# guy3540/Acoustic_Locating_VQ-VAE

Measured on AMD Instinct MI355X. Metric: spectrograms/sec (train step), speech VQ-VAE default config, higher is better.
Workload: dtype x3mx_hb

## Files before the change

acoustic_locating_vq-vae_amd/csrc/vq.hip:

```cpp
#include "alvq_common.h"

namespace alvq {

constexpr int VQ_RB_MAX = 128;
constexpr int VQ_CT = 128;
constexpr int VQ_DK = 32;
constexpr int VQ_ES = 34;
constexpr int VQ_PARTIALS = 1024;

__host__ __device__ constexpr int vq_pad32(int x, int r) { return x + ((r - x % 32) + 32) % 32; }

__global__ __launch_bounds__(256) void row_sqnorm_kernel(const float* x, float* out, long rows, int D) {
  const int lane = threadIdx.x & 63;
  for (long r = (long)blockIdx.x * 4 + (threadIdx.x >> 6); r < rows; r += (long)gridDim.x * 4) {
    float s = 0.f;
    for (int d = lane; d < D; d += 64) {
      const float v = x[r * D + d];
      s += v * v;
    }
    s = wave_sum(s);
    if (lane == 0) out[r] = s;
  }
}

struct ArgminArgs {
  const float* x;
  const float* e;
  const float* xn;
  const float* en;
  int64_t* idx;
  float* min_dist;
  long N;
  int K, D, Dp, XSTR;
};

template <int NW>
__global__ __launch_bounds__(64 * NW, 2) void vq_argmin_f32_kernel(ArgminArgs a) {
  constexpr int NT = 64 * NW, VQ_RB = 16 * NW, EPT = VQ_CT * VQ_DK / NT, ERS = NT / 32;
  extern __shared__ __attribute__((aligned(16))) float smem[];
  float* Xs = smem;
  float* Es = smem + VQ_RB * a.XSTR;

  const int tid = threadIdx.x, lane = tid & 63, wave = tid >> 6;
  const int li = lane & 15, kq = lane >> 4;
  const long r0 = (long)blockIdx.x * VQ_RB;
  const int D = a.D, K = a.K, XSTR = a.XSTR;

  for (int e = tid; e < VQ_RB * a.Dp; e += NT) {
    const int r = e / a.Dp, d = e - r * a.Dp;
    const long row = r0 + r;
    Xs[r * XSTR + d] = (row < a.N && d < D) ? a.x[row * D + d] : 0.f;
  }

  float xn[4];
#pragma unroll
  for (int r = 0; r < 4; ++r) {
    const long row = r0 + wave * 16 + kq * 4 + r;
    xn[r] = row < a.N ? a.xn[row] : 0.f;
  }
  float best[4];
  int bidx[4];
#pragma unroll
  for (int r = 0; r < 4; ++r) {
    best[r] = __builtin_inff();
    bidx[r] = 0x7fffffff;
  }

  const int ecol = tid & 31, erow0 = tid >> 5;
  float er[EPT];
  auto load_e = [&](int k0, int d0) {
#pragma unroll
    for (int i = 0; i < EPT; ++i) {
      const int k = k0 + erow0 + ERS * i, d = d0 + ecol;
      er[i] = (k < K && d < D) ? a.e[(long)k * D + d] : 0.f;
    }
  };
  auto store_e = [&]() {
#pragma unroll
    for (int i = 0; i < EPT; ++i) Es[(erow0 + ERS * i) * VQ_ES + ecol] = er[i];
  };

  const int nd = a.Dp / VQ_DK;
  const int nkt = (K + VQ_CT - 1) / VQ_CT;
  const int total = nkt * nd;
  load_e(0, 0);
  store_e();
  __syncthreads();
  f32x4 acc[8];
  for (int it = 0; it < total; ++it) {
    const int kt = it / nd, dc = it - kt * nd;
    if (dc == 0) {
#pragma unroll
      for (int ni = 0; ni < 8; ++ni) acc[ni] = f32x4{0.f, 0.f, 0.f, 0.f};
    }
    if (it + 1 < total) {
      const int kt2 = (it + 1) / nd, dc2 = (it + 1) - kt2 * nd;
      load_e(kt2 * VQ_CT, dc2 * VQ_DK);
    }
#pragma unroll
    for (int s = 0; s < VQ_DK / 4; ++s) {
      const float af = Xs[(wave * 16 + li) * XSTR + dc * VQ_DK + s * 4 + kq];
#pragma unroll
      for (int ni = 0; ni < 8; ++ni) {
        const float bf = Es[(ni * 16 + li) * VQ_ES + s * 4 + kq];
        acc[ni] = __builtin_amdgcn_mfma_f32_16x16x4f32(af, bf, acc[ni], 0, 0, 0);
      }
    }
    if (dc == nd - 1) {
#pragma unroll
      for (int ni = 0; ni < 8; ++ni) {
        const int k = kt * VQ_CT + ni * 16 + li;
        if (k < K) {
          const float bn = a.en[k];
#pragma unroll
          for (int r = 0; r < 4; ++r) {
            const float d = (xn[r] + bn) - 2.0f * acc[ni][r];
            if (d < best[r]) {
              best[r] = d;
              bidx[r] = k;
            }
          }
        }
      }
    }
    __syncthreads();
    if (it + 1 < total) {
      store_e();
      __syncthreads();
    }
  }

#pragma unroll
  for (int o = 1; o < 16; o <<= 1) {
#pragma unroll
    for (int r = 0; r < 4; ++r) {
      const float d2 = __shfl_xor(best[r], o, 64);
      const int k2 = __shfl_xor(bidx[r], o, 64);
      if (d2 < best[r] || (d2 == best[r] && k2 < bidx[r])) {
        best[r] = d2;
        bidx[r] = k2;
      }
    }
  }
  if (li == 0) {
#pragma unroll
    for (int r = 0; r < 4; ++r) {
      const long row = r0 + wave * 16 + kq * 4 + r;
      if (row < a.N) {
        a.idx[row] = (int64_t)(bidx[r] == 0x7fffffff ? 0 : bidx[r]);
        if (a.min_dist) a.min_dist[row] = best[r];
      }
    }
  }
}

constexpr int VQR_ES = 36;
template <int ND, int RW>
__global__ __launch_bounds__(256, (ND == 8 && RW == 1) ? 3 : 2) void vq_argmin_f32_reg_kernel(ArgminArgs a) {
  __shared__ __attribute__((aligned(16))) float Es[2][VQ_CT * VQR_ES];
  const int tid = threadIdx.x, lane = tid & 63, wave = tid >> 6;
  const int li = lane & 15, kq = lane >> 4;
  const long r0 = (long)blockIdx.x * (64 * RW) + wave * (16 * RW);
  const int D = a.D, K = a.K;
  const bool vec = (D & 3) == 0;

  float xa[RW][ND * 8];
#pragma unroll
  for (int f = 0; f < RW; ++f) {
    const long row = r0 + f * 16 + li;
    const float* xr = a.x + row * D;
#pragma unroll
    for (int j = 0; j < ND * 8; ++j) {
      const int d = 4 * j + kq;
      xa[f][j] = (row < a.N && d < D) ? xr[d] : 0.f;
    }
  }
  float xn[RW][4], best[RW][4];
  int bidx[RW][4];
#pragma unroll
  for (int f = 0; f < RW; ++f)
#pragma unroll
    for (int r = 0; r < 4; ++r) {
      const long row = r0 + f * 16 + kq * 4 + r;
      xn[f][r] = row < a.N ? a.xn[row] : 0.f;
      best[f][r] = __builtin_inff();
      bidx[f][r] = 0x7fffffff;
    }

  const int c8 = tid & 7, ecode = tid >> 3;
  f32x4 er[4];
  auto load_e = [&](int kt, int dc) {
#pragma unroll
    for (int i = 0; i < 4; ++i) {
      const int k = kt * VQ_CT + ecode + 32 * i, d = dc * VQ_DK + 4 * c8;
      const float* p = a.e + (long)k * D + d;
      if (k < K && vec && d + 3 < D) er[i] = *(const f32x4*)p;
      else {
#pragma unroll
        for (int q = 0; q < 4; ++q) er[i][q] = (k < K && d + q < D) ? p[q] : 0.f;
      }
    }
  };
  auto store_e = [&](int buf) {
#pragma unroll
    for (int i = 0; i < 4; ++i)
#pragma unroll
      for (int q = 0; q < 4; ++q) Es[buf][(ecode + 32 * i) * VQR_ES + q * 8 + c8] = er[i][q];
  };

  const int nkt = (K + VQ_CT - 1) / VQ_CT;
  load_e(0, 0);
  store_e(0);
  __syncthreads();
  for (int kt = 0; kt < nkt; ++kt) {
    f32x4 acc[RW][8];
#pragma unroll
    for (int f = 0; f < RW; ++f)
#pragma unroll
      for (int ni = 0; ni < 8; ++ni) acc[f][ni] = f32x4{0.f, 0.f, 0.f, 0.f};
#pragma unroll
    for (int dc = 0; dc < ND; ++dc) {
      const bool more = !(kt == nkt - 1 && dc == ND - 1);
      if (more) load_e(dc == ND - 1 ? kt + 1 : kt, dc == ND - 1 ? 0 : dc + 1);
      const float* eb = &Es[dc & 1][li * VQR_ES + kq * 8];
#pragma unroll
      for (int half = 0; half < 2; ++half) {
        f32x4 b0[4], b1[4];
#pragma unroll
        for (int n4 = 0; n4 < 4; ++n4) {
          const float* p = eb + (half * 4 + n4) * 16 * VQR_ES;
          b0[n4] = *(const f32x4*)p;
          b1[n4] = *(const f32x4*)(p + 4);
        }
#pragma unroll
        for (int s = 0; s < 8; ++s)
#pragma unroll
          for (int n4 = 0; n4 < 4; ++n4) {
            const float bf = s < 4 ? b0[n4][s & 3] : b1[n4][s & 3];
#pragma unroll
            for (int f = 0; f < RW; ++f)
              acc[f][half * 4 + n4] = __builtin_amdgcn_mfma_f32_16x16x4f32(xa[f][dc * 8 + s], bf, acc[f][half * 4 + n4], 0, 0, 0);
          }
      }
      if (more) store_e((dc + 1) & 1);
      __syncthreads();
    }
#pragma unroll
    for (int ni = 0; ni < 8; ++ni) {
      const int k = kt * VQ_CT + ni * 16 + li;
      if (k < K) {
        const float bn = a.en[k];
#pragma unroll
        for (int f = 0; f < RW; ++f)
#pragma unroll
          for (int r = 0; r < 4; ++r) {
            const float d = (xn[f][r] + bn) - 2.0f * acc[f][ni][r];
            if (d < best[f][r]) {
              best[f][r] = d;
              bidx[f][r] = k;
            }
          }
      }
    }
  }
#pragma unroll
  for (int o = 1; o < 16; o <<= 1)
#pragma unroll
    for (int f = 0; f < RW; ++f)
#pragma unroll
      for (int r = 0; r < 4; ++r) {
        const float d2 = __shfl_xor(best[f][r], o, 64);
        const int k2 = __shfl_xor(bidx[f][r], o, 64);
        if (d2 < best[f][r] || (d2 == best[f][r] && k2 < bidx[f][r])) {
          best[f][r] = d2;
          bidx[f][r] = k2;
        }
      }
  if (li == 0) {
#pragma unroll
    for (int f = 0; f < RW; ++f)
#pragma unroll
      for (int r = 0; r < 4; ++r) {
        const long row = r0 + f * 16 + kq * 4 + r;
        if (row < a.N) {
          a.idx[row] = (int64_t)(bidx[f][r] == 0x7fffffff ? 0 : bidx[f][r]);
          if (a.min_dist) a.min_dist[row] = best[f][r];
        }
      }
  }
}

__global__ __launch_bounds__(256) void vq_gather_loss_kernel(const float* x, const float* e, const int64_t* idx,
                                                             float* q_st, float* partials, int32_t* hist, long N, int K,
                                                             int D) {
  const int lane = threadIdx.x & 63, wave = threadIdx.x >> 6;
  extern __shared__ int lhist[];
  const bool use_lds = hist && K <= 8192;
  if (use_lds) {
    for (int k = threadIdx.x; k < K; k += 256) lhist[k] = 0;
    __syncthreads();
  }
  const long per = (N + gridDim.x - 1) / gridDim.x;
  const long rb = (long)blockIdx.x * per, re = rb + per < N ? rb + per : N;
  float s = 0.f;
  for (long r = rb + wave; r < re; r += 4) {
    const long k = idx[r];
    for (int d = lane; d < D; d += 64) {
      const float xv = x[r * D + d];
      const float diff = e[k * D + d] - xv;
      q_st[r * D + d] = xv + diff;
      s += diff * diff;
    }
    if (lane == 0 && hist) atomicAdd(use_lds ? &lhist[k] : &hist[k], 1);
  }
  if (use_lds) {
    __syncthreads();
    for (int k = threadIdx.x; k < K; k += 256)
      if (lhist[k]) atomicAdd(&hist[k], lhist[k]);
  }
  __shared__ float red[4];
  s = block_sum<kPairwise4, false>(s, red);
  if (threadIdx.x == 0) partials[blockIdx.x] = s;
}

template <bool QLAT>
__global__ __launch_bounds__(256) void vq_finalize_kernel(const float* partials, int nparts, const int32_t* hist,
                                                          float* out, long N, int K, int D, float beta) {
  __shared__ float red[256];
  const int t = threadIdx.x;
  float s = 0.f;
  for (int i = t; i < nparts; i += 256) s += partials[i];
  const float sq = tree256_sum<true>(s, red);
  float h = 0.f;
  for (int k = t; k < K; k += 256) {
    const float p = (float)hist[k] / (float)N;
    h += p * logf(p + 1e-10f);
  }
  h = tree256_sum<false>(h, red);
  if (t == 0) {
    const float m = sq / (float)((double)N * (double)D);
    out[0] = QLAT ? m + beta * m : beta * m;
    out[1] = expf(-h);
  }
}

__global__ __launch_bounds__(256) void vq_backward_dx_kernel(const float* g, const float* grad_loss, const float* x,
                                                             const float* e, const int64_t* idx, float* dx, long N, int D,
                                                             float cx) {
  const int lane = threadIdx.x & 63, wave = threadIdx.x >> 6;
  const float sx = (grad_loss ? grad_loss[0] : 1.f) * cx;
  for (long r = (long)blockIdx.x * 4 + wave; r < N; r += (long)gridDim.x * 4) {
    const long k = idx[r];
    for (int d = lane; d < D; d += 64) {
      const float diff = e[k * D + d] - x[r * D + d];
      dx[r * D + d] = (g ? g[r * D + d] : 0.f) - sx * diff;
    }
  }
}

constexpr int VQL_CAP = 2048;
constexpr int VQL_CHUNK = 1024;
template <int VEC>
__global__ __launch_bounds__(256) void vq_codebook_grad_kernel(const float* grad_loss, const float* x, const float* e,
                                                               const int64_t* idx, float* partial, long N, int K, int D,
                                                               long rows_per_part, float ce) {
  typedef float vec_t __attribute__((ext_vector_type(VEC)));
  __shared__ int list[VQL_CAP];
  __shared__ int wave_tot[4];
  __shared__ vec_t comb[256];
  const int k = blockIdx.x, part = blockIdx.y, tid = threadIdx.x;
  const float se = (grad_loss ? grad_loss[0] : 1.f) * ce;
  const int TD = D / VEC;
  const int G = 256 / TD;
  const int grp = tid / TD, ld = tid - grp * TD;
  const bool summer = grp < G;
  vec_t ek, acc;
#pragma unroll
  for (int v = 0; v < VEC; ++v) {
    ek[v] = summer ? e[(long)k * D + ld * VEC + v] : 0.f;
    acc[v] = 0.f;
  }
  int nlist = 0;
  auto flush = [&]() {
    if (!summer) return;
    int i = grp;
    for (; i + G < nlist; i += 2 * G) {
      const vec_t a = *(const vec_t*)(x + (long)list[i] * D + ld * VEC);
      const vec_t b = *(const vec_t*)(x + (long)list[i + G] * D + ld * VEC);
      acc += se * (ek - a);
      acc += se * (ek - b);
    }
    if (i < nlist) acc += se * (ek - *(const vec_t*)(x + (long)list[i] * D + ld * VEC));
  };
  const long rbeg = (long)part * rows_per_part;
  const long rend = rbeg + rows_per_part < N ? rbeg + rows_per_part : N;
  for (long base = rbeg; base < rend; base += VQL_CHUNK) {
    int mine[4], cnt = 0;
#pragma unroll
    for (int j = 0; j < 4; ++j) {
      const long r = base + 4 * tid + j;
      if (r < rend && idx[r] == k) mine[cnt++] = (int)r;
    }
    int total;
    const int pos = nlist + block_scan_excl<false>(cnt, wave_tot, total);
    for (int j = 0; j < cnt; ++j) list[pos + j] = mine[j];
    nlist += total;
    __syncthreads();
    if (nlist > VQL_CAP - VQL_CHUNK) {
      flush();
      nlist = 0;
      __syncthreads();
    }
  }
  flush();
  comb[tid] = acc;
  __syncthreads();
  if (tid < TD) {
    vec_t s = comb[tid];
    for (int g = 1; g < G; ++g) s += comb[g * TD + tid];
    *(vec_t*)(partial + ((long)part * K + k) * D + tid * VEC) = s;
  }
}

__global__ __launch_bounds__(256) void vq_codebook_grad_reduce_kernel(const float* partial, float* dE, long kd, int P) {
  for (long i = (long)blockIdx.x * 256 + threadIdx.x; i < kd; i += (long)gridDim.x * 256) {
    float s = 0.f;
    for (int p = 0; p < P; ++p) s += partial[(long)p * kd + i];
    dE[i] += s;
  }
}

__global__ __launch_bounds__(256) void onehot_kernel(const int64_t* idx, float* enc, long N, int K) {
  const long total = N * (long)K;
  for (long e = (long)blockIdx.x * 256 + threadIdx.x; e < total; e += (long)gridDim.x * 256) {
    const long r = e / K;
    const int k = (int)(e - r * K);
    enc[e] = (idx[r] == k) ? 1.f : 0.f;
  }
}

}

using namespace alvq;

static int grid_for(long work_items, int per_block) {
  long g = (work_items + per_block - 1) / per_block;
  if (g > 2048) g = 2048;
  if (g < 1) g = 1;
  return (int)g;
}

extern "C" int64_t alvq_vq_argmin_workspace_bytes(int64_t N, int K, int D) {
  if (N <= 0 || K <= 0 || D <= 0) return -1;
  return (int64_t)(N + K) * (int64_t)sizeof(float);
}

extern "C" int alvq_vq_argmin_f32(const float* x, const float* codebook, int64_t* idx, float* min_dist,
                                  void* workspace, int64_t N, int K, int D, void* stream) {
  ALVQ_REQUIRE(x && codebook && idx && workspace, ALVQ_EINVAL, "alvq_vq_argmin_f32: null pointer");
  ALVQ_REQUIRE(N > 0 && K > 0 && D > 0, ALVQ_EINVAL, "alvq_vq_argmin_f32: bad dims N=%ld K=%d D=%d", (long)N, K, D);
  ALVQ_REQUIRE(D <= 512, ALVQ_EUNSUPPORTED, "alvq_vq_argmin_f32: D=%d > 512 does not fit the stationary LDS tile", D);
  ALVQ_REQUIRE(N / 64 < (1L << 31) - 2, ALVQ_EUNSUPPORTED, "alvq_vq_argmin_f32: N too large");
  hipStream_t s = (hipStream_t)stream;
  float* xn = (float*)workspace;
  float* en = xn + N;
  hipLaunchKernelGGL(row_sqnorm_kernel, dim3(grid_for(N, 4)), dim3(256), 0, s, x, xn, (long)N, D);
  hipLaunchKernelGGL(row_sqnorm_kernel, dim3(grid_for(K, 4)), dim3(256), 0, s, codebook, en, (long)K, D);
  const int Dp = (D + VQ_DK - 1) / VQ_DK * VQ_DK;
  const int XSTR = vq_pad32(Dp, 2);
  ArgminArgs a{x, codebook, xn, en, idx, min_dist, (long)N, K, D, Dp, XSTR};
  static DeviceOnce attr_set;
  if (attr_set.need()) {
    (void)hipFuncSetAttribute((const void*)vq_argmin_f32_kernel<4>, hipFuncAttributeMaxDynamicSharedMemorySize, 160 * 1024);
    (void)hipFuncSetAttribute((const void*)vq_argmin_f32_kernel<8>, hipFuncAttributeMaxDynamicSharedMemorySize, 160 * 1024);
  }
  if (D <= 256 && option(OPT_VQ_REG) != 0) {
    const int nd = D <= 64 ? 2 : (D <= 128 ? 4 : 8);
    const bool two = nd != 8 && N >= 128L * 512;
    const int rows_wg = two ? 128 : 64;
    const dim3 grid((unsigned)((N + rows_wg - 1) / rows_wg));
    if (nd == 2 && two) hipLaunchKernelGGL((vq_argmin_f32_reg_kernel<2, 2>), grid, dim3(256), 0, s, a);
    else if (nd == 2) hipLaunchKernelGGL((vq_argmin_f32_reg_kernel<2, 1>), grid, dim3(256), 0, s, a);
    else if (nd == 4 && two) hipLaunchKernelGGL((vq_argmin_f32_reg_kernel<4, 2>), grid, dim3(256), 0, s, a);
    else if (nd == 4) hipLaunchKernelGGL((vq_argmin_f32_reg_kernel<4, 1>), grid, dim3(256), 0, s, a);
    else hipLaunchKernelGGL((vq_argmin_f32_reg_kernel<8, 1>), grid, dim3(256), 0, s, a);
    return check_launch("alvq_vq_argmin_f32");
  }
  const bool wide = D >= 128 && (size_t)(128 * XSTR + VQ_CT * VQ_ES) * sizeof(float) <= 160 * 1024;
  const int rb = wide ? 128 : 64;
  const size_t lds = (size_t)(rb * XSTR + VQ_CT * VQ_ES) * sizeof(float);
  const dim3 grid((unsigned)((N + rb - 1) / rb));
  if (wide) hipLaunchKernelGGL(vq_argmin_f32_kernel<8>, grid, dim3(512), lds, s, a);
  else hipLaunchKernelGGL(vq_argmin_f32_kernel<4>, grid, dim3(256), lds, s, a);
  return check_launch("alvq_vq_argmin_f32");
}

extern "C" int alvq_vq_gather_loss_f32(const float* x, const float* codebook, const int64_t* idx, float* q_st,
                                       float* sq_partials, int32_t* hist, int64_t N, int K, int D, void* stream) {
  ALVQ_REQUIRE(x && codebook && idx && q_st && sq_partials, ALVQ_EINVAL, "alvq_vq_gather_loss_f32: null pointer");
  ALVQ_REQUIRE(N > 0 && K > 0 && D > 0, ALVQ_EINVAL, "alvq_vq_gather_loss_f32: bad dims");
  hipLaunchKernelGGL(vq_gather_loss_kernel, dim3(VQ_PARTIALS), dim3(256), (hist && K <= 8192) ? K * sizeof(int) : 0,
                     (hipStream_t)stream, x, codebook, idx, q_st, sq_partials, hist, (long)N, K, D);
  return check_launch("alvq_vq_gather_loss_f32");
}

extern "C" int alvq_vq_finalize_f32(const float* sq_partials, const int32_t* hist, float* out, int64_t N, int K, int D,
                                    float beta, void* stream) {
  ALVQ_REQUIRE(sq_partials && hist && out, ALVQ_EINVAL, "alvq_vq_finalize_f32: null pointer");
  ALVQ_REQUIRE(N > 0 && K > 0 && D > 0, ALVQ_EINVAL, "alvq_vq_finalize_f32: bad dims");
  hipLaunchKernelGGL(vq_finalize_kernel<true>, dim3(1), dim3(256), 0, (hipStream_t)stream, sq_partials, VQ_PARTIALS, hist,
                     out, (long)N, K, D, beta);
  return check_launch("alvq_vq_finalize_f32");
}

extern "C" int alvq_vq_finalize_ema_f32(const float* sq_partials, const int32_t* hist, float* out, int64_t N, int K, int D,
                                        float beta, void* stream) {
  ALVQ_REQUIRE(sq_partials && hist && out, ALVQ_EINVAL, "alvq_vq_finalize_ema_f32: null pointer");
  ALVQ_REQUIRE(N > 0 && K > 0 && D > 0, ALVQ_EINVAL, "alvq_vq_finalize_ema_f32: bad dims");
  hipLaunchKernelGGL(vq_finalize_kernel<false>, dim3(1), dim3(256), 0, (hipStream_t)stream, sq_partials, VQ_PARTIALS, hist,
                     out, (long)N, K, D, beta);
  return check_launch("alvq_vq_finalize_ema_f32");
}

constexpr int VQ_PARTS_MAX = 16;

static int vq_parts(int64_t N) {
  int64_t p = N / 4096;
  return p < 1 ? 1 : (p > VQ_PARTS_MAX ? VQ_PARTS_MAX : (int)p);
}

extern "C" int64_t alvq_vq_backward_workspace_bytes(int K, int D) {
  return (K <= 0 || D <= 0) ? -1 : (int64_t)VQ_PARTS_MAX * K * D * (int64_t)sizeof(float);
}

extern "C" int alvq_vq_backward_f32(const float* g, const float* grad_loss, const float* x, const float* codebook,
                                    const int64_t* idx, float* dx, float* dE, void* workspace, int64_t N, int K, int D,
                                    float beta, void* stream) {
  ALVQ_REQUIRE(x && codebook && idx && (dx || dE), ALVQ_EINVAL, "alvq_vq_backward_f32: null pointer");
  ALVQ_REQUIRE(N > 0 && K > 0 && D > 0, ALVQ_EINVAL, "alvq_vq_backward_f32: bad dims");
  ALVQ_REQUIRE(!dE || workspace, ALVQ_EINVAL, "alvq_vq_backward_f32: the codebook gradient needs the workspace");
  ALVQ_REQUIRE(N < (1L << 31) && K <= 65535 && ((D % 4 == 0 && D <= 512) || D <= 256), ALVQ_EUNSUPPORTED,
               "alvq_vq_backward_f32: N=%ld K=%d D=%d outside the supported range", (long)N, K, D);
  const double nd = (double)N * (double)D;
  hipStream_t s = (hipStream_t)stream;
  if (dx)
    hipLaunchKernelGGL(vq_backward_dx_kernel, dim3(grid_for(N, 4)), dim3(256), 0, s, g, grad_loss, x, codebook, idx, dx,
                       (long)N, D, (float)(2.0 * beta / nd));
  if (dE) {
    const int P = vq_parts(N);
    const long rpp = ((N + P - 1) / P + VQL_CHUNK - 1) / VQL_CHUNK * VQL_CHUNK;
    float* partial = (float*)workspace;
    if (D % 4 == 0)
      hipLaunchKernelGGL(vq_codebook_grad_kernel<4>, dim3(K, P), dim3(256), 0, s, grad_loss, x, codebook, idx, partial, (long)N,
                         K, D, rpp, (float)(2.0 / nd));
    else
      hipLaunchKernelGGL(vq_codebook_grad_kernel<1>, dim3(K, P), dim3(256), 0, s, grad_loss, x, codebook, idx, partial, (long)N,
                         K, D, rpp, (float)(2.0 / nd));
    hipLaunchKernelGGL(vq_codebook_grad_reduce_kernel, dim3(grid_for((long)K * D, 256)), dim3(256), 0, s,
                       (const float*)partial, dE, (long)K * D, P);
  }
  return check_launch("alvq_vq_backward_f32");
}

extern "C" int alvq_onehot_f32(const int64_t* idx, float* encodings, int64_t N, int K, void* stream) {
  ALVQ_REQUIRE(idx && encodings, ALVQ_EINVAL, "alvq_onehot_f32: null pointer");
  ALVQ_REQUIRE(N > 0 && K > 0, ALVQ_EINVAL, "alvq_onehot_f32: bad dims");
  hipLaunchKernelGGL(onehot_kernel, dim3(grid_for(N * (long)K, 256 * 8)), dim3(256), 0, (hipStream_t)stream, idx,
                     encodings, (long)N, K);
  return check_launch("alvq_onehot_f32");
}
```

acoustic_locating_vq-vae_amd/csrc/wgrad_reduce.h:

```cpp
#pragma once
#include "alvq_common.h"

namespace alvq {

static __device__ __forceinline__ void wgrad_reduce_body(const float* partial, float* dw, int splits, int KW, int M, int C,
                                                         int w_layout, int accumulate, const float* scale, long stride, int bid,
                                                         int nblk) {
  const long total = (long)KW * M * C;
  const float sc = scale ? *scale : 1.f;
  if (w_layout == ALVQ_W_OIK && KW == 3) {
    const long pairs = (long)M * C;
    for (long q = bid * 256L + threadIdx.x; q < pairs; q += (long)nblk * 256) {
      float s0 = 0.f, s1 = 0.f, s2 = 0.f;
      const float* p = partial + q;
      int k = 0;
      for (; k + 2 <= splits; k += 2) {
        const float* pa = p + (long)k * stride;
        const float* pb = pa + stride;
        const float a0 = pa[0], a1 = pa[pairs], a2 = pa[2 * pairs], b0 = pb[0], b1 = pb[pairs], b2 = pb[2 * pairs];
        s0 = (s0 + a0) + b0;
        s1 = (s1 + a1) + b1;
        s2 = (s2 + a2) + b2;
      }
      for (; k < splits; ++k) {
        const float* pa = p + (long)k * stride;
        s0 += pa[0];
        s1 += pa[pairs];
        s2 += pa[2 * pairs];
      }
      if (scale) { s0 *= sc; s1 *= sc; s2 *= sc; }
      float* o = dw + 3 * q;
      if (accumulate) { s0 += o[0]; s1 += o[1]; s2 += o[2]; }
      o[0] = s0; o[1] = s1; o[2] = s2;
    }
    return;
  }
  for (long e = bid * 256L + threadIdx.x; e < total; e += (long)nblk * 256) {
    int m, c, t;
    if (w_layout == ALVQ_W_OIK) {
      t = (int)(e % KW);
      c = (int)((e / KW) % C);
      m = (int)(e / ((long)KW * C));
    } else {
      const int tt = (int)(e % KW);
      t = KW - 1 - tt;
      m = (int)((e / KW) % M);
      c = (int)(e / ((long)KW * M));
    }
    const long src = ((long)t * M + m) * C + c;
    float s = 0.f;
    int k = 0;
    for (; k + 4 <= splits; k += 4) {
      const float v0 = partial[(long)k * stride + src], v1 = partial[(long)(k + 1) * stride + src],
                  v2 = partial[(long)(k + 2) * stride + src], v3 = partial[(long)(k + 3) * stride + src];
      s = (((s + v0) + v1) + v2) + v3;
    }
    for (; k < splits; ++k) s += partial[(long)k * stride + src];
    if (scale) s *= sc;
    dw[e] = accumulate ? dw[e] + s : s;
  }
}
static __global__ void wgrad_reduce_kernel(const float* partial, float* dw, int splits, int KW, int M, int C, int w_layout,
                                    int accumulate, const float* scale) {
  wgrad_reduce_body(partial, dw, splits, KW, M, C, w_layout, accumulate, scale, (long)KW * M * C, blockIdx.x, gridDim.x);
}

template <int RB>
static __device__ __forceinline__ void wgrad_reduce_iok_body(float (&tile)[3][RB][65], const float* partial, float* dw, int splits,
                                                             int KW, int M, int C, int accumulate, const float* scale, int bid) {
  constexpr int RI = RB / 8;
  const int ctiles = (C + 63) / 64;
  const int m0 = (bid / ctiles) * RB, c0 = (bid % ctiles) * 64;
  const int tx = threadIdx.x & 31, ty = threadIdx.x >> 5;
  const long plane = (long)M * C, total = (long)KW * plane;
  const bool pair = (C % 2 == 0);
  float s0[3][RI], s1[3][RI];
#pragma unroll
  for (int t = 0; t < 3; ++t)
#pragma unroll
    for (int i = 0; i < RI; ++i) s0[t][i] = s1[t][i] = 0.f;
  const int c = c0 + 2 * tx;
  const bool full = pair && m0 + RB <= M && c0 + 64 <= C;
  if (full) {
    const float* p0 = partial + (long)(m0 + ty) * C + c;
    if (KW == 3) {
#pragma unroll 4
      for (int k = 0; k < splits; ++k) {
        float2 v[3][RI];
#pragma unroll
        for (int t = 0; t < 3; ++t)
#pragma unroll
          for (int i = 0; i < RI; ++i) v[t][i] = *(const float2*)(p0 + (long)k * total + (long)t * plane + (long)(8 * i) * C);
#pragma unroll
        for (int t = 0; t < 3; ++t)
#pragma unroll
          for (int i = 0; i < RI; ++i) {
            s0[t][i] += v[t][i].x;
            s1[t][i] += v[t][i].y;
          }
      }
    } else {
#pragma unroll 4
      for (int k = 0; k < splits; ++k) {
        float2 v[RI];
#pragma unroll
        for (int i = 0; i < RI; ++i) v[i] = *(const float2*)(p0 + (long)k * total + (long)(8 * i) * C);
#pragma unroll
        for (int i = 0; i < RI; ++i) {
          s0[0][i] += v[i].x;
          s1[0][i] += v[i].y;
        }
      }
    }
  } else
  for (int k = 0; k < splits; ++k) {
    const float* pk = partial + (long)k * total + c;
#pragma unroll
    for (int t = 0; t < 3; ++t) {
      if (t >= KW) break;
#pragma unroll
      for (int i = 0; i < RI; ++i) {
        const int m = m0 + ty + 8 * i;
        if (m >= M) continue;
        const float* p = pk + (long)t * plane + (long)m * C;
        if (pair && c + 1 < C) {
          const float2 v = *(const float2*)p;
          s0[t][i] += v.x;
          s1[t][i] += v.y;
        } else {
          if (c < C) s0[t][i] += p[0];
          if (c + 1 < C) s1[t][i] += p[1];
        }
      }
    }
  }
#pragma unroll
  for (int t = 0; t < 3; ++t) {
    if (t >= KW) break;
#pragma unroll
    for (int i = 0; i < RI; ++i) {
      tile[t][ty + 8 * i][2 * tx] = s0[t][i];
      tile[t][ty + 8 * i][2 * tx + 1] = s1[t][i];
    }
  }
  __syncthreads();
  const int run = RB * KW;
  for (int e = threadIdx.x; e < 64 * run; e += 256) {
    const int cc = e / run, j = e - cc * run, mr = j / KW, tt = j - mr * KW;
    if (c0 + cc >= C || m0 + mr >= M) continue;
    const long o = ((long)(c0 + cc) * M + m0) * KW + j;
    float v = tile[KW - 1 - tt][mr][cc];
    if (scale) v *= *scale;
    dw[o] = accumulate ? dw[o] + v : v;
  }
}
template <int RB>
static __global__ __launch_bounds__(256) void wgrad_reduce_iok_kernel(const float* partial, float* dw, int splits, int KW,
                                                                      int M, int C, int accumulate, const float* scale) {
  __shared__ float tile[3][RB][65];
  wgrad_reduce_iok_body<RB>(tile, partial, dw, splits, KW, M, C, accumulate, scale, blockIdx.x);
}

static inline void wgrad_reduce_launch(const float* partial, float* dw, int splits, int KW, int M, int C, int w_layout,
                                       int accumulate, hipStream_t s, const float* scale = nullptr) {
  if (w_layout == ALVQ_W_IOK) {
    const int grid = ((M + 15) / 16) * ((C + 63) / 64);
    hipLaunchKernelGGL(wgrad_reduce_iok_kernel<16>, dim3(grid), dim3(256), 0, s, partial, dw, splits, KW, M, C, accumulate, scale);
    return;
  }
  const long total = (long)KW * M * C;
  int rgrid = (int)((total + 255) / 256);
  if (rgrid > 2048) rgrid = 2048;
  hipLaunchKernelGGL(wgrad_reduce_kernel, dim3(rgrid), dim3(256), 0, s, partial, dw, splits, KW, M, C, w_layout, accumulate, scale);
}

}
```

acoustic_locating_vq-vae_amd/csrc/wgrad_reduce_batch.hip:

```cpp
#include "alvq_common.h"
#include "wgrad_reduce.h"

namespace alvq {

constexpr int RB_MAX = 40;
struct ReduceBatch {
  alvq_reduce_desc d[RB_MAX];
  int blk0[RB_MAX];
  int nblk[RB_MAX];
  int n;
};

__global__ __launch_bounds__(256) void wgrad_reduce_batch_kernel(ReduceBatch b) {
  __shared__ float tile[3][16][65];
  int di = 0;
  for (int i = 1; i < b.n; ++i)
    if ((int)blockIdx.x >= b.blk0[i]) di = i;
  const alvq_reduce_desc& d = b.d[di];
  const int lb = blockIdx.x - b.blk0[di];
  const int acc = d.accumulate;
  if (d.w_layout == ALVQ_W_IOK && d.stride == (int64_t)d.KW * d.M * d.C)
    wgrad_reduce_iok_body<16>(tile, d.partial, d.dst, d.splits, d.KW, d.M, d.C, acc, d.scale, lb);
  else
    wgrad_reduce_body(d.partial, d.dst, d.splits, d.KW, d.M, d.C, d.w_layout, acc, d.scale, (long)d.stride, lb, b.nblk[di]);
}

}

using namespace alvq;

extern "C" int alvq_wgrad_reduce_batch(const alvq_reduce_desc* descs, int n, void* stream) {
  ALVQ_REQUIRE(descs && n > 0, ALVQ_EINVAL, "alvq_wgrad_reduce_batch: no descriptors");
  for (int i = 0; i < n; ++i) {
    const alvq_reduce_desc& s = descs[i];
    ALVQ_REQUIRE(s.partial && s.dst, ALVQ_EINVAL, "alvq_wgrad_reduce_batch: null pointer in descriptor %d", i);
    ALVQ_REQUIRE(s.splits >= 1 && s.splits <= 64 && s.M > 0 && s.C > 0 && (s.KW == 1 || s.KW == 3), ALVQ_EINVAL,
                 "alvq_wgrad_reduce_batch: bad dims in descriptor %d", i);
    ALVQ_REQUIRE(s.w_layout == ALVQ_W_OIK || s.w_layout == ALVQ_W_IOK, ALVQ_EINVAL, "alvq_wgrad_reduce_batch: w_layout in descriptor %d", i);
    ALVQ_REQUIRE(s.stride >= (int64_t)s.KW * s.M * s.C, ALVQ_EINVAL, "alvq_wgrad_reduce_batch: stride in descriptor %d", i);
  }
  for (int i0 = 0; i0 < n; i0 += RB_MAX) {
    ReduceBatch b{};
    b.n = n - i0 < RB_MAX ? n - i0 : RB_MAX;
    int blocks = 0;
    for (int i = 0; i < b.n; ++i) {
      const alvq_reduce_desc& s = descs[i0 + i];
      b.d[i] = s;
      const long total = (long)s.KW * s.M * s.C;
      int nb;
      if (s.w_layout == ALVQ_W_IOK && s.stride == total) nb = ((s.M + 15) / 16) * ((s.C + 63) / 64);
      else {
        nb = (int)((total + 255) / 256);
        if (nb > 2048) nb = 2048;
      }
      b.blk0[i] = blocks;
      b.nblk[i] = nb;
      blocks += nb;
    }
    hipLaunchKernelGGL(wgrad_reduce_batch_kernel, dim3(blocks), dim3(256), 0, (hipStream_t)stream, b);
    int rc = check_launch("alvq_wgrad_reduce_batch");
    if (rc) return rc;
  }
  return ALVQ_OK;
}
```

Before: 7454.

## Vectorize weight-gradient split reductions and prefetch VQ codebook indices

Adds float4 vectorized paths to the weight-gradient split reduction for OIK layouts (KW 3 and 1) and for the IOK tiled reduction, batching loads across several splits to increase memory-level parallelism. The IOK path also loads the old dw values before the reduction so the accumulate read overlaps it. In the VQ codebook gradient kernel, the flush loop is unrolled 8-way and the index loads for the next chunk are software-prefetched. Costs are higher register pressure and extra alignment-conditional code paths.

```diff
diff --git a/acoustic_locating_vq-vae_amd/csrc/vq.hip b/acoustic_locating_vq-vae_amd/csrc/vq.hip
--- a/acoustic_locating_vq-vae_amd/csrc/vq.hip
+++ b/acoustic_locating_vq-vae_amd/csrc/vq.hip
@@ -384,6 +384,13 @@
   auto flush = [&]() {
     if (!summer) return;
     int i = grp;
+    for (; i + 7 * G < nlist; i += 8 * G) {
+      vec_t a[8];
+#pragma unroll
+      for (int j = 0; j < 8; ++j) a[j] = *(const vec_t*)(x + (long)list[i + j * G] * D + ld * VEC);
+#pragma unroll
+      for (int j = 0; j < 8; ++j) acc += se * (ek - a[j]);
+    }
     for (; i + G < nlist; i += 2 * G) {
       const vec_t a = *(const vec_t*)(x + (long)list[i] * D + ld * VEC);
       const vec_t b = *(const vec_t*)(x + (long)list[i + G] * D + ld * VEC);
@@ -394,13 +401,23 @@
   };
   const long rbeg = (long)part * rows_per_part;
   const long rend = rbeg + rows_per_part < N ? rbeg + rows_per_part : N;
-  for (long base = rbeg; base < rend; base += VQL_CHUNK) {
-    int mine[4], cnt = 0;
+  auto load_idx = [&](long (&v)[4], long base) {
 #pragma unroll
     for (int j = 0; j < 4; ++j) {
       const long r = base + 4 * tid + j;
-      if (r < rend && idx[r] == k) mine[cnt++] = (int)r;
-    }
+      v[j] = r < rend ? idx[r] : -1L;
+    }
+  };
+  long cur[4], nxt[4];
+  load_idx(nxt, rbeg);
+  for (long base = rbeg; base < rend; base += VQL_CHUNK) {
+#pragma unroll
+    for (int j = 0; j < 4; ++j) cur[j] = nxt[j];
+    load_idx(nxt, base + VQL_CHUNK);
+    int mine[4], cnt = 0;
+#pragma unroll
+    for (int j = 0; j < 4; ++j)
+      if (cur[j] == k) mine[cnt++] = (int)(base + 4 * tid + j);
     int total;
     const int pos = nlist + block_scan_excl<false>(cnt, wave_tot, total);
     for (int j = 0; j < cnt; ++j) list[pos + j] = mine[j];
diff --git a/acoustic_locating_vq-vae_amd/csrc/wgrad_reduce.h b/acoustic_locating_vq-vae_amd/csrc/wgrad_reduce.h
--- a/acoustic_locating_vq-vae_amd/csrc/wgrad_reduce.h
+++ b/acoustic_locating_vq-vae_amd/csrc/wgrad_reduce.h
@@ -3,11 +3,83 @@
 
 namespace alvq {
 
+
+static inline int wgrad_reduce_vec_ok(const float* partial, const float* dw, int w_layout, int M, int C, long stride) {
+  return w_layout == ALVQ_W_OIK && ((long)M * C) % 4 == 0 && stride % 4 == 0 && ((uintptr_t)partial | (uintptr_t)dw) % 16 == 0;
+}
+static inline int wgrad_reduce_blocks(int KW, int M, int C, int vec) {
+  const long items = vec ? (long)M * C / 4 : (long)KW * M * C;
+  const long nb = (items + 255) / 256;
+  return nb > 2048 ? 2048 : (nb < 1 ? 1 : (int)nb);
+}
+
+template <int NK, int KW>
+static __device__ __forceinline__ void wgrad_reduce_add4(f32x4 (&s)[KW], const float* p, long stride, long plane) {
+  f32x4 v[NK][KW];
+#pragma unroll
+  for (int j = 0; j < NK; ++j)
+#pragma unroll
+    for (int t = 0; t < KW; ++t) v[j][t] = *(const f32x4*)(p + j * stride + t * plane);
+#pragma unroll
+  for (int j = 0; j < NK; ++j)
+#pragma unroll
+    for (int t = 0; t < KW; ++t) s[t] += v[j][t];
+}
+template <int KW>
+static __device__ __forceinline__ void wgrad_reduce_sum4(f32x4 (&s)[KW], const float* p, int splits, long stride, long plane) {
+#pragma unroll
+  for (int t = 0; t < KW; ++t) s[t] = f32x4{0.f, 0.f, 0.f, 0.f};
+  constexpr int NK = KW == 3 ? 4 : 8;
+  int k = 0;
+  for (; k + NK <= splits; k += NK) wgrad_reduce_add4<NK, KW>(s, p + (long)k * stride, stride, plane);
+  if (NK == 8 && k + 4 <= splits) {
+    wgrad_reduce_add4<4, KW>(s, p + (long)k * stride, stride, plane);
+    k += 4;
+  }
+  const float* pk = p + (long)k * stride;
+  switch (splits - k) {
+    case 3: wgrad_reduce_add4<3, KW>(s, pk, stride, plane); break;
+    case 2: wgrad_reduce_add4<2, KW>(s, pk, stride, plane); break;
+    case 1: wgrad_reduce_add4<1, KW>(s, pk, stride, plane); break;
+    default: break;
+  }
+}
+
 static __device__ __forceinline__ void wgrad_reduce_body(const float* partial, float* dw, int splits, int KW, int M, int C,
                                                          int w_layout, int accumulate, const float* scale, long stride, int bid,
-                                                         int nblk) {
+                                                         int nblk, int vec) {
   const long total = (long)KW * M * C;
   const float sc = scale ? *scale : 1.f;
+  if (vec && w_layout == ALVQ_W_OIK && KW == 3) {
+    const long pairs = (long)M * C, quads = pairs / 4;
+    for (long q = bid * 256L + threadIdx.x; q < quads; q += (long)nblk * 256) {
+      f32x4* o = (f32x4*)(dw + 12 * q);
+      f32x4 d0, d1, d2;
+      if (accumulate) { d0 = o[0]; d1 = o[1]; d2 = o[2]; }
+      f32x4 s[3];
+      wgrad_reduce_sum4<3>(s, partial + 4 * q, splits, stride, pairs);
+      if (scale) { s[0] *= sc; s[1] *= sc; s[2] *= sc; }
+      f32x4 r0 = {s[0][0], s[1][0], s[2][0], s[0][1]}, r1 = {s[1][1], s[2][1], s[0][2], s[1][2]},
+            r2 = {s[2][2], s[0][3], s[1][3], s[2][3]};
+      if (accumulate) { r0 += d0; r1 += d1; r2 += d2; }
+      o[0] = r0; o[1] = r1; o[2] = r2;
+    }
+    return;
+  }
+  if (vec && w_layout == ALVQ_W_OIK && KW == 1) {
+    const long quads = total / 4;
+    for (long q = bid * 256L + threadIdx.x; q < quads; q += (long)nblk * 256) {
+      f32x4* o = (f32x4*)(dw + 4 * q);
+      f32x4 d0;
+      if (accumulate) d0 = o[0];
+      f32x4 s[1];
+      wgrad_reduce_sum4<1>(s, partial + 4 * q, splits, stride, total);
+      if (scale) s[0] *= sc;
+      if (accumulate) s[0] += d0;
+      o[0] = s[0];
+    }
+    return;
+  }
   if (w_layout == ALVQ_W_OIK && KW == 3) {
     const long pairs = (long)M * C;
     for (long q = bid * 256L + threadIdx.x; q < pairs; q += (long)nblk * 256) {
@@ -61,8 +133,8 @@
   }
 }
 static __global__ void wgrad_reduce_kernel(const float* partial, float* dw, int splits, int KW, int M, int C, int w_layout,
-                                    int accumulate, const float* scale) {
-  wgrad_reduce_body(partial, dw, splits, KW, M, C, w_layout, accumulate, scale, (long)KW * M * C, blockIdx.x, gridDim.x);
+                                    int accumulate, const float* scale, int vec) {
+  wgrad_reduce_body(partial, dw, splits, KW, M, C, w_layout, accumulate, scale, (long)KW * M * C, blockIdx.x, gridDim.x, vec);
 }
 
 template <int RB>
@@ -74,6 +146,36 @@
   const int tx = threadIdx.x & 31, ty = threadIdx.x >> 5;
   const long plane = (long)M * C, total = (long)KW * plane;
   const bool pair = (C % 2 == 0);
+  const int run = RB * KW;
+  constexpr int NOUT = 64 * RB * 3 / 256;
+  float old[NOUT];
+  if (accumulate) {
+#pragma unroll
+    for (int i = 0; i < NOUT; ++i) {
+      const int e = threadIdx.x + 256 * i;
+      if (e >= 64 * run) break;
+      const int cc = e / run, j = e - cc * run, mr = j / KW;
+      if (c0 + cc < C && m0 + mr < M) old[i] = dw[((long)(c0 + cc) * M + m0) * KW + j];
+    }
+  }
+  if (C % 4 == 0 && (uintptr_t)partial % 16 == 0 && m0 + RB <= M && c0 + 64 <= C) {
+    static_assert(RB % 16 == 0, "16 tile rows per pass of 256 threads");
+    const int tx4 = threadIdx.x & 15, ty4 = threadIdx.x >> 4;
+#pragma unroll
+    for (int i = 0; i < RB / 16; ++i) {
+      const int row = ty4 + 16 * i;
+      const float* p = partial + (long)(m0 + row) * C + c0 + 4 * tx4;
+      f32x4 s[3];
+      if (KW == 3) wgrad_reduce_sum4<3>(s, p, splits, total, plane);
+      else wgrad_reduce_sum4<1>(*(f32x4(*)[1])&s, p, splits, total, plane);
+#pragma unroll
+      for (int t = 0; t < 3; ++t) {
+        if (t >= KW) break;
+#pragma unroll
+        for (int j = 0; j < 4; ++j) tile[t][row][4 * tx4 + j] = s[t][j];
+      }
+    }
+  } else {
   float s0[3][RI], s1[3][RI];
 #pragma unroll
   for (int t = 0; t < 3; ++t)
@@ -143,15 +245,18 @@
       tile[t][ty + 8 * i][2 * tx + 1] = s1[t][i];
     }
   }
+  }
   __syncthreads();
-  const int run = RB * KW;
-  for (int e = threadIdx.x; e < 64 * run; e += 256) {
+#pragma unroll
+  for (int i = 0; i < NOUT; ++i) {
+    const int e = threadIdx.x + 256 * i;
+    if (e >= 64 * run) break;
     const int cc = e / run, j = e - cc * run, mr = j / KW, tt = j - mr * KW;
     if (c0 + cc >= C || m0 + mr >= M) continue;
     const long o = ((long)(c0 + cc) * M + m0) * KW + j;
     float v = tile[KW - 1 - tt][mr][cc];
     if (scale) v *= *scale;
-    dw[o] = accumulate ? dw[o] + v : v;
+    dw[o] = accumulate ? old[i] + v : v;
   }
 }
 template <int RB>
@@ -168,10 +273,9 @@
     hipLaunchKernelGGL(wgrad_reduce_iok_kernel<16>, dim3(grid), dim3(256), 0, s, partial, dw, splits, KW, M, C, accumulate, scale);
     return;
   }
-  const long total = (long)KW * M * C;
-  int rgrid = (int)((total + 255) / 256);
-  if (rgrid > 2048) rgrid = 2048;
-  hipLaunchKernelGGL(wgrad_reduce_kernel, dim3(rgrid), dim3(256), 0, s, partial, dw, splits, KW, M, C, w_layout, accumulate, scale);
-}
-
-}
+  const int vec = wgrad_reduce_vec_ok(partial, dw, w_layout, M, C, (long)KW * M * C);
+  const int rgrid = wgrad_reduce_blocks(KW, M, C, vec);
+  hipLaunchKernelGGL(wgrad_reduce_kernel, dim3(rgrid), dim3(256), 0, s, partial, dw, splits, KW, M, C, w_layout, accumulate, scale, vec);
+}
+
+}
diff --git a/acoustic_locating_vq-vae_amd/csrc/wgrad_reduce_batch.hip b/acoustic_locating_vq-vae_amd/csrc/wgrad_reduce_batch.hip
--- a/acoustic_locating_vq-vae_amd/csrc/wgrad_reduce_batch.hip
+++ b/acoustic_locating_vq-vae_amd/csrc/wgrad_reduce_batch.hip
@@ -8,6 +8,7 @@
   alvq_reduce_desc d[RB_MAX];
   int blk0[RB_MAX];
   int nblk[RB_MAX];
+  unsigned char vec[RB_MAX];
   int n;
 };
 
@@ -22,7 +23,7 @@
   if (d.w_layout == ALVQ_W_IOK && d.stride == (int64_t)d.KW * d.M * d.C)
     wgrad_reduce_iok_body<16>(tile, d.partial, d.dst, d.splits, d.KW, d.M, d.C, acc, d.scale, lb);
   else
-    wgrad_reduce_body(d.partial, d.dst, d.splits, d.KW, d.M, d.C, d.w_layout, acc, d.scale, (long)d.stride, lb, b.nblk[di]);
+    wgrad_reduce_body(d.partial, d.dst, d.splits, d.KW, d.M, d.C, d.w_layout, acc, d.scale, (long)d.stride, lb, b.nblk[di], b.vec[di]);
 }
 
 }
@@ -50,8 +51,8 @@
       int nb;
       if (s.w_layout == ALVQ_W_IOK && s.stride == total) nb = ((s.M + 15) / 16) * ((s.C + 63) / 64);
       else {
-        nb = (int)((total + 255) / 256);
-        if (nb > 2048) nb = 2048;
+        b.vec[i] = (unsigned char)wgrad_reduce_vec_ok(s.partial, s.dst, s.w_layout, s.M, s.C, (long)s.stride);
+        nb = wgrad_reduce_blocks(s.KW, s.M, s.C, b.vec[i]);
       }
       b.blk0[i] = blocks;
       b.nblk[i] = nb;
```

New measurement: 7452. Within noise of the previous version (-0.0%).
